# clancylian/retinaface

Hardware: AMD Instinct MI355X
Metric: faces/sec (higher is better)
Workload: dtype f16; 1 GPU; mnet25 fp16 HIP, 448x448, batch 8 per GPU (BASELINE.json configs[1], the metric point); global_batch=8, parallelism=dp1 (image sharding, no data-path collective), tickets_in_flight=96, lanes=3, steps_coalesced_per_launch=32, input=ring of 768 distinct frames per GPU (462 MB, HBM-resident)

## Files before the change

### retinaface_amd/csrc/kernels.hip

```cpp
#include "kernels.h"

#include <atomic>
#include <type_traits>

#include "pack.h"

namespace rf {

typedef float f32x4 __attribute__((ext_vector_type(4)));
typedef _Float16 f16x8 __attribute__((ext_vector_type(8)));

typedef signed char i8x16 __attribute__((ext_vector_type(16)));
typedef int i32x4 __attribute__((ext_vector_type(4)));

template <typename T> struct Vec;
template <> struct Vec<half_t> { static constexpr int N = 8; typedef f16x8 type; };
template <> struct Vec<float> { static constexpr int N = 4; typedef f32x4 type; };
template <> struct Vec<int8_t> { static constexpr int N = 16; typedef i8x16 type; };

template <typename T> __device__ __forceinline__ T to_T(float v);
template <> __device__ __forceinline__ half_t to_T<half_t>(float v) { return (half_t)v; }
template <> __device__ __forceinline__ float to_T<float>(float v) { return v; }
template <> __device__ __forceinline__ int8_t to_T<int8_t>(float v) { return (int8_t)(int)fminf(fmaxf(rintf(v), -127.f), 127.f); }

// ... 2497 lines not shown
    const int lh = L.h, lw = L.w_, hh = lh >> 1, wh = lw >> 1;
    const int n_my = first < ntiles ? (ntiles - 1 - first) / G + 1 : 0;
    const TileStep step(G, L.tiles_x, L.tiles_y);
    auto halo_of = [&](int b) -> T * { return (T *)(smem + (size_t)b * W::BUF_BYTES); };
    auto aux_of = [&](int b) -> T * { return (T *)(smem + (size_t)b * W::BUF_BYTES + W::L_BYTES); };

    int kl[LPW], kc[CPW];
    const int in_ld = L.in_ld;
#pragma unroll
    for (int j = 0; j < LPW; j++) {
        const int s = (wave + 4 * j) * 64 + lane;
        const int row = s / W::CPR, rem = s % W::CPR;
        const int px = rem / W::CPP, ch = rem % W::CPP;
        const bool real = row < HR && px < HC && ch < DPP;
        kl[j] = real ? ((((row * lw + px) * in_ld + ch * VEC) * (int)sizeof(T)) | (px << 26)) : (int)(63u << 26);
    }
#pragma unroll
    for (int j = 0; j < CPW; j++) {
        const int s = (wave + 4 * j) * 64 + lane;
        const int cpix = s / DPP, ch = s % DPP;
        const int cy = cpix / CW, cx = cpix % CW;
        kc[j] = (((cy * wh + cx) * CIN + ch * VEC) * (int)sizeof(T)) | (cx << 26);
    }
    const unsigned lat_bytes = (unsigned)(lh * lw * in_ld - L.in_off) * (unsigned)sizeof(T);
    const unsigned up_bytes = (unsigned)(hh * wh * CIN) * (unsigned)sizeof(T);
    const T *in = L.in + L.in_off;
    auto dma = [&](int tx, int ty, int img, int b) {
        const auto rs = image_rsrc(in + (size_t)img * lh * lw * in_ld, lat_bytes);
        const auto ru = image_rsrc(L.up + (size_t)img * hh * wh * CIN, up_bytes);
        const int iy0 = ty * TH - 1, ix0 = tx * TW - 1;
        const int sbase = (iy0 * lw + ix0) * in_ld * (int)sizeof(T);
        unsigned char *hd = (unsigned char *)halo_of(b), *cd = (unsigned char *)aux_of(b);
#pragma unroll
        for (int j = 0; j < LPW; j++) {
            const int piece = wave + 4 * j;
            const int dx = (int)((unsigned)kl[j] >> 26);
            const unsigned off = (dx != 63 && (unsigned)(ix0 + dx) < (unsigned)lw) ? (unsigned)((kl[j] & 0x03ffffff) + sbase) : kOobOffset;
            if (piece < W::PIECES && piece * 64 + lane < W::SLOTS) lds_dma16(rs, hd + piece * 1024, off);
        }
        const int cy0 = ty * (TH / 2) - 2, cx0 = tx * (TW / 2) - 2;
        const int cbase = (cy0 * wh + cx0) * CIN * (int)sizeof(T);
#pragma unroll
        for (int j = 0; j < CPW; j++) {
            const int piece = wave + 4 * j;
            const int cx = (int)((unsigned)kc[j] >> 26);
            const unsigned off = (unsigned)(cx0 + cx) < (unsigned)wh ? (unsigned)((kc[j] & 0x03ffffff) + cbase) : kOobOffset;
            if (piece < W::CPIECES) lds_dma16(ru, cd + piece * 1024, off);
        }
    };
    T *out0 = L.out0;
    const int ld0 = L.ld0, off0 = L.off0;
    auto store_tile = [&](int b, int img, int oy0, int ox0) {
        constexpr int OPV = 64 / VEC;
        const T *s_res = aux_of(b);
        const auto r0 = image_rsrc(out0 + (size_t)img * lh * lw * ld0 + off0, (unsigned)(lh * lw * ld0 - off0) * (unsigned)sizeof(T));
        const int pbase = oy0 * lw + ox0;
        V v[SPW];
#pragma unroll
        for (int m = 0; m < SPW; m++) { const int i = tid + m * kThreads; v[m] = *(const V *)(s_res + (i / OPV) * LDO + (i % OPV) * VEC); }
#pragma unroll
        for (int m = 0; m < SPW; m++) {
            const int i = tid + m * kThreads;
            const int p = i / OPV, c = (i % OPV) * VEC;
            const int py = p / TW, px = p % TW;
            buf_store16(r0, ox0 + px < lw ? (unsigned)(((pbase + py * lw + px) * ld0 + c) * (int)sizeof(T)) : kOobOffset, v[m]);
        }
    };

    const int wn = wave;
    Frag wst[1][KCH];
    {
        const Frag *wsrc = (const Frag *)L.w + (size_t)wn * KCH * 64 + lane;
#pragma unroll
        for (int kc2 = 0; kc2 < KCH; kc2++) wst[0][kc2] = wsrc[kc2 * 64];
    }
    const f32x4 bias = *(const f32x4 *)(L.b + acc_cout(wn, lane, 0));
    const f32x4 mult = load_mult(L.m, acc_cout(wn, lane, 0));
    const float a_lat = L.a_lat, a_up = L.a_up;
    const bool int_blend = L.int_blend != 0;
    int pbase[NJ];
#pragma unroll
    for (int j = 0; j < NJ; j++) {
        const int p = acc_pixel(j, lane);
        pbase[j] = (p / TW) * ROWP + (p % TW) * LDI;
    }
    int b_lat[W::NBL], b_c0[W::NBL], b_step[W::NBL], b_yx[W::NBL];
#pragma unroll
    for (int m = 0; m < W::NBL; m++) {
        int i = tid + m * 256;
        const bool real = i < HR * HC * DPP;
        i = real ? i : 0;
        const int pix = i / DPP, cv = i % DPP;
        const int dy = pix / HC, dx = pix % HC;
        const int ly = 2 + ((dy - 1) >> 1), lx = 2 + ((dx - 1) >> 1);
        const int sy = ((dy - 1) & 1) ? 1 : -1, sx = ((dx - 1) & 1) ? 1 : -1;
        b_lat[m] = dy * ROWP + dx * LDI + cv * VEC;
        b_c0[m] = (ly * CW + lx) * CIN + cv * VEC;
        b_step[m] = (sy * CW * CIN) * 65536 + (sx * CIN + 32768);
        b_yx[m] = real ? (dy << 8 | dx) : -1;
    }
    __builtin_amdgcn_s_waitcnt(0x0F70);

    TileCoord cur(first, L.tiles_x, L.tiles_y), pf = cur;
#pragma unroll
    for (int d = 0; d < DIST; d++)
        if (d < n_my) { dma(pf.tx, pf.ty, pf.img, d); step.advance(pf); }
    wait_vmcnt<0>();
    lds_barrier();
    int p_img = 0, p_oy0 = 0, p_ox0 = 0;
    for (int k = 0; k < n_my; k++) {
        const int b = k % NBUF;
        const bool st = k > 0, ld = k + DIST < n_my;
        T *s_in_b = halo_of(b);
        T *s_x = aux_of(b);
        const int iy0 = cur.ty * TH - 1, ix0 = cur.tx * TW - 1;
        if (st) store_tile((k - 1) % NBUF, p_img, p_oy0, p_ox0);
        p_img = cur.img; p_oy0 = cur.ty * TH; p_ox0 = cur.tx * TW;
        step.advance(cur);
#pragma unroll
        for (int m = 0; m < W::NBL; m++) {
            if (b_yx[m] < 0) continue;
            const int rs_ = b_step[m] >> 16, cs_ = (b_step[m] & 0xffff) - 32768;
            const V lat = *(const V *)(s_in_b + b_lat[m]);
            const V u0 = *(const V *)(s_x + b_c0[m]), u1 = *(const V *)(s_x + b_c0[m] + cs_);
            const V u2 = *(const V *)(s_x + b_c0[m] + rs_), u3 = *(const V *)(s_x + b_c0[m] + rs_ + cs_);
            const bool ok = (unsigned)(iy0 + (b_yx[m] >> 8)) < (unsigned)lh && (unsigned)(ix0 + (b_yx[m] & 0xff)) < (unsigned)lw;
            *(V *)(s_in_b + b_lat[m]) = upadd_blend<T>(lat, u0, u1, u2, u3, ok, int_blend, a_lat, a_up);
        }
        lds_barrier();
        if (ld) { dma(pf.tx, pf.ty, pf.img, (k + DIST) % NBUF); step.advance(pf); }
        typename M::Acc acc[1][NJ];
#pragma unroll
        for (int j = 0; j < NJ; j++) acc[0][j] = acc_init<T>(bias);
        gemm_stationary<T, 1, NJ, KCH, DEPTH, true>(acc, wst, [&](int j, int kc2) -> Frag {
            const int kb = kc2 * M::K + (lane >> 4) * M::KPL;
            const int tap = kb / CIN, c = kb % CIN;
            const int koff = (tap / 3) * ROWP + (tap % 3) * LDI + c;
            return kb < KTOT ? *(const Frag *)(s_in_b + pbase[j] + koff) : M::zero();
        });
#pragma unroll
        for (int j = 0; j < NJ; j++) store_acc<T, LDO>(s_x, mult, bias, acc[0][j], wn, j, lane, true);
        wait_vmcnt<0>();
        lds_barrier();
    }
    if (n_my > 0) store_tile((n_my - 1) % NBUF, p_img, p_oy0, p_ox0);
}


template <typename T>
static void conv3_ws_launch(hipStream_t s, Conv3Args<T> &a, int nlv, int total_tiles) {
    typedef Conv3WsCfg<T> W;
    auto kern = conv3x3_ws_kernel<T>;
    static std::atomic<int> resident_cache[kMaxDevices] = {};
    const int resident = kernel_residency(resident_cache, kern, W::LDS_BYTES);
    const int want = persistent_grid(total_tiles, resident);
    int grid = 0;
    for (int l = 0; l < 3; l++) {
        Conv3Level<T> &L = a.lv[l];
        if (l >= nlv) { L.gb_begin = 0x7fffffff; L.gsz = 1; L.ntiles = 0; continue; }
        long g = want == total_tiles ? L.ntiles : ((long)L.ntiles * want + total_tiles - 1) / total_tiles;
        if (g < 1) g = 1;
        if (g > L.ntiles) g = L.ntiles;
        L.gb_begin = grid;
        L.gsz = (int)g;
        grid += (int)g;
    }
    hipLaunchKernelGGL(kern, dim3(grid), dim3(kThreads), W::LDS_BYTES, s, a);
}

template <typename T, int CIN, int COUT, int TH, int TW, bool UPADD, bool PADROW>
static void conv3_launch(hipStream_t s, Conv3Args<T> &a, int nlv, int total_tiles) {
    typedef Conv3Cfg<T, CIN, COUT, TH, TW, PADROW> C;
    if constexpr (sizeof(T) <= 2 && CIN == 64 && COUT == 48 && TH == 8 && TW == 8 && !UPADD && PADROW) {
        bool split32 = true;
        for (int l = 0; l < nlv; l++) split32 = split32 && a.lv[l].n0 == 32 && a.lv[l].out1 != nullptr;
        if constexpr (sizeof(T) == 2) {
            if (split32) { conv3_ws_launch<T>(s, a, nlv, total_tiles); return; }
        }
    }
    auto kern = conv3x3_kernel<T, CIN, COUT, TH, TW, UPADD, PADROW>;
    static std::atomic<int> resident_cache[kMaxDevices] = {};
    const int resident = kernel_residency(resident_cache, kern, C::LDS_BYTES);
    const int want = sizeof(T) <= 2 ? persistent_grid(total_tiles, resident) : total_tiles;
    int grid = 0;
    for (int l = 0; l < 3; l++) {
        Conv3Level<T> &L = a.lv[l];
        if (l >= nlv) { L.gb_begin = 0x7fffffff; L.gsz = 1; L.ntiles = 0; continue; }
        long g = want == total_tiles ? L.ntiles : ((long)L.ntiles * want + total_tiles - 1) / total_tiles;
        if (g < 1) g = 1;
        if (g > L.ntiles) g = L.ntiles;
        L.gb_begin = grid;
        L.gsz = (int)g;
        grid += (int)g;
    }
    hipLaunchKernelGGL(kern, dim3(grid), dim3(kThreads), C::LDS_BYTES, s, a);
}

template <typename T, int CIN, int COUT, int TH, int TW, bool PADROW = false>
static TileInfo conv3_dispatch(hipStream_t s, const Conv3Params<T> *p, int nlv, int h, int w) {
    typedef Conv3Cfg<T, CIN, COUT, TH, TW, PADROW> C;
    TileInfo ti{TH, TW, C::LDS_BYTES, ((w + TW - 1) / TW) * ((h + TH - 1) / TH)};
    if (!p) return ti;
    Conv3Args<T> a;
    int total = 0;
    for (int l = 0; l < 3; l++) {
        const Conv3Params<T> &q = p[l < nlv ? l : nlv - 1];
        int tiles_x = (q.w_ + TW - 1) / TW, tiles_y = (q.h + TH - 1) / TH;
        a.lv[l] = Conv3Level<T>{q.in, q.up, q.w, q.b, q.m, q.out0, q.out1, q.in_ld, q.in_off, q.ld0, q.off0, q.n0, q.ld1, q.off1,
                                q.h, q.w_, tiles_x, tiles_y, q.n * tiles_x * tiles_y, 0, 1, q.a_lat, q.a_up,
                                (sizeof(T) == 1 && q.a_lat == 1.f && q.a_up == 1.f && !q.blend_fp32) ? 1 : 0};
        if (l < nlv) total += q.n * tiles_x * tiles_y;
    }
    if (p[0].up) {
        if constexpr (CIN == 64 && COUT == 64) conv3_launch<T, CIN, COUT, TH, TW, true, PADROW>(s, a, nlv, total);
        else throw LaunchUnsupported("fused upsample + add: only the 64 -> 64 aggregation conv has a kernel instance");
    } else {
        conv3_launch<T, CIN, COUT, TH, TW, false, PADROW>(s, a, nlv, total);
    }
    return ti;
}

template <typename T>
static void conv3_up_ws_launch(hipStream_t s, const Conv3Params<T> &q) {
    typedef Conv3UpWsCfg<T> W;
    auto kern = conv3x3_up_dma_kernel<T>;
    static std::atomic<int> resident_cache[kMaxDevices] = {};
    const int dev = launch_device();
    int resident = resident_cache[dev].load(std::memory_order_acquire);
    if (!resident) {
        set_max_lds(kern, W::LDS_BYTES);
        int nb = 0;
        if (hipOccupancyMaxActiveBlocksPerMultiprocessor(&nb, (const void *)kern, kThreads, W::LDS_BYTES) != hipSuccess || nb < 1) nb = 1;
        resident = nb;
        resident_cache[dev].store(resident, std::memory_order_release);
    }
    const int tiles_x = (q.w_ + 7) / 8, tiles_y = (q.h + 7) / 8;
    Conv3Args<T> a;
    for (int l = 0; l < 3; l++)
        a.lv[l] = Conv3Level<T>{q.in, q.up, q.w, q.b, q.m, q.out0, q.out1, q.in_ld, q.in_off, q.ld0, q.off0, q.n0, q.ld1, q.off1,
                                q.h, q.w_, tiles_x, tiles_y, q.n * tiles_x * tiles_y, 0, 1, q.a_lat, q.a_up,
                                (sizeof(T) == 1 && q.a_lat == 1.f && q.a_up == 1.f && !q.blend_fp32) ? 1 : 0};
    const int total = q.n * tiles_x * tiles_y;
    if (total == 0) return;
    a.lv[0].gsz = persistent_grid(total, resident);
    hipLaunchKernelGGL(kern, dim3(a.lv[0].gsz), dim3(kThreads), W::LDS_BYTES, s, a);
}

template <typename T>
static TileInfo conv3_select(hipStream_t s, const Conv3Params<T> *p, int nlv, int cin, int cout, int h, int w) {
    if constexpr (sizeof(T) <= 2) {
        const bool up_ws = sizeof(T) == 2 && p && (long)p[0].h * p[0].w_ >= 48 * 48;
        if (p && nlv == 1 && p[0].up && cin == 64 && cout == 64 && up_ws && p[0].h % 2 == 0 && p[0].w_ % 2 == 0 &&
            p[0].n0 == 64 && p[0].in_ld == 64) {
            conv3_up_ws_launch<T>(s, p[0]);
            return TileInfo{8, 8, Conv3UpWsCfg<T>::LDS_BYTES, ((w + 7) / 8) * ((h + 7) / 8)};
        }
        if (cin == 64 && cout == 64) return conv3_dispatch<T, 64, 64, 4, 8, true>(s, p, nlv, h, w);
        if (cin == 64 && cout == 48) return conv3_dispatch<T, 64, 48, 8, 8, true>(s, p, nlv, h, w);
        return TileInfo{0, 0, 0, 0};
    }
    else {
        const bool small = nlv == 1 && (size_t)h * w <= 32 * 32;
        if (cin == 64 && cout == 64)
            return conv3_dispatch<T, 64, 64, 4, 8>(s, p, nlv, h, w);
        if (cin == 16 && cout == 32)
            return small ? conv3_dispatch<T, 16, 32, 4, 8>(s, p, nlv, h, w) : conv3_dispatch<T, 16, 32, 8, 8>(s, p, nlv, h, w);
        if (cin == 64 && cout == 48) return conv3_dispatch<T, 64, 48, 8, 8>(s, p, nlv, h, w);
        if (cin == 16 && cout == 16) return conv3_dispatch<T, 16, 16, 8, 8>(s, p, nlv, h, w);
    }
    return TileInfo{0, 0, 0, 0};
}

template <typename T> void launch_conv3x3(hipStream_t s, const Conv3Params<T> *levels, int nlevels) {
    if (nlevels < 1 || nlevels > 3) throw LaunchUnsupported("conv3x3: 1..3 levels per launch");
    for (int l = 1; l < nlevels; l++)
        if (levels[l].cin != levels[0].cin || levels[l].cout != levels[0].cout || levels[l].up)
            throw LaunchUnsupported("conv3x3: the levels of one launch must share (cin, cout) and have no fused upsample");
    TileInfo ti = conv3_select<T>(s, levels, nlevels, levels[0].cin, levels[0].cout, levels[0].h, levels[0].w_);
    if (ti.th == 0) throw LaunchUnsupported("no 3x3 kernel instance for this (cin, cout)");
}
template <typename T> TileInfo conv3x3_tile_info(int cin, int cout, int h, int w) {
    return conv3_select<T>(nullptr, nullptr, 1, cin, cout, h, w);
}
template void launch_conv3x3<half_t>(hipStream_t, const Conv3Params<half_t> *, int);
template void launch_conv3x3<float>(hipStream_t, const Conv3Params<float> *, int);
template void launch_conv3x3<int8_t>(hipStream_t, const Conv3Params<int8_t> *, int);
template TileInfo conv3x3_tile_info<half_t>(int, int, int, int);
template TileInfo conv3x3_tile_info<float>(int, int, int, int);
template TileInfo conv3x3_tile_info<int8_t>(int, int, int, int);

template <typename T> struct SshTailCfg {
    typedef Mma<T> M;
    static constexpr int VEC = Vec<T>::N;
    static constexpr int TH = 8, TW = 8, P = TH * TW;
    static constexpr int R1 = TW + 2, N1 = (TH + 2) * R1, PT1 = (N1 + 15) / 16;
    static constexpr int HC = TW + 4, NH = (TH + 4) * HC;
    static constexpr int LDI = lds_row<T>(16);
    static constexpr int LDO = lds_row<T>(32);
    static constexpr int KTOT = 9 * 16, KCH = (KTOT + M::K - 1) / M::K;
    static constexpr int CPV = 16 / VEC;
    static constexpr int STAGE_ITEMS = NH * CPV, NPF = (STAGE_ITEMS + kThreads - 1) / kThreads;
    static constexpr size_t IN_BYTES = sizeof(T) * (size_t)(NH * LDI), MID_BYTES = sizeof(T) * (size_t)(PT1 * 16 * LDI),
                            OUT_BYTES = sizeof(T) * (size_t)(P * LDO);
    static constexpr size_t LDS_BYTES = IN_BYTES + MID_BYTES + 2 * OUT_BYTES;
    static_assert(IN_BYTES % 16 == 0 && MID_BYTES % 16 == 0, "LDS carve must stay 16-byte aligned");
    static constexpr int OCC = 4;
};

template <typename T>
struct SshTailLevel {
    const T *in; const T *wb; const float *bb; const float *mb; const T *wc; const float *bc; const float *mc; T *cat;
    int h, w_, tiles_x, tiles_y, ntiles, gb_begin, gsz;
};
template <typename T> struct SshTailArgs { SshTailLevel<T> lv[3]; };

template <typename T, typename ACC>
__device__ __forceinline__ uint2 pack_acc(f32x4 mult, f32x4 bv, ACC acc) {
    uint2 h = {0u, 0u};
    if constexpr (sizeof(T) == 2) {
        h.x = pack_f16((float)acc[0], (float)acc[1], true);
        h.y = pack_f16((float)acc[2], (float)acc[3], true);
    } else {
        static_assert(sizeof(T) == 1, "fp16 / int8 engines only");
#pragma unroll
        for (int r = 0; r < 4; r++)
            h.x = __builtin_amdgcn_cvt_pk_u8_f32(RF_RNDNE(__builtin_amdgcn_fmed3f(fmaf((float)acc[r], mult[r], bv[r]), 0.f, 127.f)), r, h.x);
    }
    return h;
}
template <typename T> __device__ __forceinline__ void store_packed4(T *dst, uint2 h) {
    if constexpr (sizeof(T) == 2) *(uint2 *)dst = h;
    else *(uint32_t *)dst = h.x;
}

template <typename T>
__global__ __launch_bounds__(kThreads, SshTailCfg<T>::OCC) void ssh_tail_kernel(SshTailArgs<T> a) {
    typedef SshTailCfg<T> C;
    typedef typename Vec<T>::type V;
    typedef Mma<T> M;
    typedef typename M::Frag Frag;
    constexpr int VEC = C::VEC, TH = C::TH, TW = C::TW, P = C::P, R1 = C::R1, N1 = C::N1, PT1 = C::PT1, HC = C::HC;
    constexpr int LDI = C::LDI, LDO = C::LDO, KTOT = C::KTOT, KCH = C::KCH, CPV = C::CPV, NPF = C::NPF;
    extern __shared__ __attribute__((aligned(16))) unsigned char smem[];
    T *s_in = (T *)smem;
    T *s_mid = (T *)(smem + C::IN_BYTES);
    T *s_out = (T *)(smem + C::IN_BYTES + C::MID_BYTES);

    const int tid = threadIdx.x, lane = tid & 63, wave = tid >> 6;
    const int gbid = xcd_remap(blockIdx.x, gridDim.x);
    const int lvl = (gbid >= a.lv[1].gb_begin ? 1 : 0) + (gbid >= a.lv[2].gb_begin ? 1 : 0);
    const SshTailLevel<T> &L = a.lv[lvl];
    const int first = gbid - L.gb_begin, G = L.gsz, ntiles = L.ntiles;
    const int lh = L.h, lw = L.w_;
    const int kg = lane >> 4;

    const int ctb = wave & 1, ptb0 = wave >> 1;
    Frag wb[1][KCH], wc[1][KCH];
    {
        const Frag *sb = (const Frag *)L.wb + (size_t)ctb * KCH * 64 + lane, *sc = (const Frag *)L.wc + lane;
#pragma unroll
        for (int kc = 0; kc < KCH; kc++) { wb[0][kc] = sb[kc * 64]; wc[0][kc] = sc[kc * 64]; }
    }
    const f32x4 bias_b = *(const f32x4 *)(L.bb + acc_cout(ctb, lane, 0)), mult_b = load_mult(L.mb, acc_cout(ctb, lane, 0));
    const f32x4 bias_c = *(const f32x4 *)(L.bc + acc_cout(0, lane, 0)), mult_c = load_mult(L.mc, acc_cout(0, lane, 0));

    int pb1[4], ryx1[4];
#pragma unroll
    for (int i = 0; i < 4; i++) {
        const int pt = ptb0 + 2 * i;
        int p = pt * 16 + (lane & 15);
        const bool real = pt < PT1 && p < N1;
        p = real ? p : N1 - 1;
        const int ry = p / R1, rx = p % R1;
        pb1[i] = (ry * HC + rx) * LDI;
        ryx1[i] = real ? (ry << 8 | rx) : -1;
    }
    const int p2 = wave * 16 + (lane & 15);
    const int pb2 = ((p2 / TW) * R1 + p2 % TW) * LDI;

    V pre[NPF];
    int koff[NPF], kdx[NPF];
#pragma unroll
    for (int k = 0; k < NPF; k++) {
        int i = tid + k * kThreads;
        i = i < C::STAGE_ITEMS ? i : C::STAGE_ITEMS - 1;
        const int pix = i / CPV, cv = i % CPV;
        koff[k] = (((pix / HC) * lw + pix % HC) * 16 + cv * VEC) * (int)sizeof(T);
        kdx[k] = pix % HC;
    }
    const unsigned in_img_bytes = (unsigned)(lh * lw * 16) * (unsigned)sizeof(T);
    auto fetch = [&](int tx, int ty, int img) {
        const auto rs = image_rsrc(L.in + (size_t)img * lh * lw * 16, in_img_bytes);
        const int iy0 = ty * TH - 2, ix0 = tx * TW - 2;
        const int sbase = (iy0 * lw + ix0) * 16 * (int)sizeof(T);
#pragma unroll
        for (int k = 0; k < NPF; k++) {
            const unsigned off = (unsigned)(ix0 + kdx[k]) < (unsigned)lw ? (unsigned)(koff[k] + sbase) : kOobOffset;
            pre[k] = buf_load16<V>(rs, off);
        }
    };
    auto store_tile = [&](const T *s_res, int img, int oy0, int ox0) {
        constexpr int OPV = 32 / VEC;
        const auto ro = image_rsrc(L.cat + (size_t)img * lh * lw * 64 + 32, (unsigned)(lh * lw * 64 - 32) * (unsigned)sizeof(T));
        const int pbase = oy0 * lw + ox0;
        for (int i = tid; i < P * OPV; i += kThreads) {
            const int p = i / OPV, cv = i % OPV;
            const int py = p / TW, px = p % TW;
            const unsigned off = ox0 + px < lw ? (unsigned)(((pbase + py * lw + px) * 64 + cv * VEC) * (int)sizeof(T)) : kOobOffset;
            buf_store16(ro, off, *(const V *)(s_res + p * LDO + cv * VEC));
        }
    };
    const TileStep step(G, L.tiles_x, L.tiles_y);
    TileCoord cur(first, L.tiles_x, L.tiles_y), nxt = cur;
    step.advance(nxt);
    if (first < ntiles) fetch(cur.tx, cur.ty, cur.img);
    __builtin_amdgcn_s_waitcnt(0x0F70);

    auto xf_tap = [&](int kc, int rowp) -> int {
        const int kb = kc * M::K + kg * M::KPL;
        const int tap = kb / 16, c = kb % 16;
        return kb < KTOT ? (tap / 3) * rowp + (tap % 3) * LDI + c : -1;
    };

    int p_img = -1, p_oy0 = 0, p_ox0 = 0;
    int buf = 0;
    constexpr int O_ELEMS = (int)(C::OUT_BYTES / sizeof(T));
    for (int t = first; t < ntiles; t += G) {
        const int oy0 = cur.ty * TH, ox0 = cur.tx * TW, img = cur.img;
        T *const s_out_b = s_out + buf * O_ELEMS;
#pragma unroll
        for (int k = 0; k < NPF; k++) {
            const int i = tid + k * kThreads;
            if (i < C::STAGE_ITEMS) *(V *)(s_in + (i / CPV) * LDI + (i % CPV) * VEC) = pre[k];
        }
        if (t + G < ntiles) fetch(nxt.tx, nxt.ty, nxt.img);
        cur = nxt;
        step.advance(nxt);
        __syncthreads();
        if (p_img >= 0) store_tile(s_out + (buf ^ 1) * O_ELEMS, p_img, p_oy0, p_ox0);
        p_img = img; p_oy0 = oy0; p_ox0 = ox0;

#pragma unroll
        for (int half = 0; half < 2; half++) {
            typename M::Acc acc[1][2];
#pragma unroll
            for (int j = 0; j < 2; j++) acc[0][j] = acc_init<T>(bias_b);
            gemm_stationary<T, 1, 2, KCH, 2>(acc, wb, [&](int j, int kc) -> Frag {
                const int o = xf_tap(kc, HC * LDI);
                return o >= 0 ? *(const Frag *)(s_in + pb1[2 * half + j] + o) : M::zero();
            });
#pragma unroll
            for (int jj = 0; jj < 2; jj++) {
                const int j = 2 * half + jj;
                if (ryx1[j] < 0) continue;
                const int ry = ryx1[j] >> 8, rx = ryx1[j] & 0xff;
                const uint2 h = pack_acc<T>(mult_b, bias_b, acc[0][jj]);
                if (ctb == 0) {
                    if ((unsigned)(ry - 1) < (unsigned)TH && (unsigned)(rx - 1) < (unsigned)TW)
                        store_packed4<T>(s_out_b + ((ry - 1) * TW + rx - 1) * LDO + kg * 4, h);
                } else {
                    const int y = oy0 - 1 + ry, x = ox0 - 1 + rx;
                    const bool inside = (unsigned)y < (unsigned)lh && (unsigned)x < (unsigned)lw;
                    const uint2 z = {0u, 0u};
                    store_packed4<T>(s_mid + (ry * R1 + rx) * LDI + kg * 4, inside ? h : z);
                }
            }
        }
        __syncthreads();

        {
            typename M::Acc acc[1][1];
            acc[0][0] = acc_init<T>(bias_c);
            gemm_stationary<T, 1, 1, KCH, 2>(acc, wc, [&](int, int kc) -> Frag {
                const int o = xf_tap(kc, R1 * LDI);
                return o >= 0 ? *(const Frag *)(s_mid + pb2 + o) : M::zero();
            });
            store_packed4<T>(s_out_b + p2 * LDO + 16 + kg * 4, pack_acc<T>(mult_c, bias_c, acc[0][0]));
        }
        buf ^= 1;
    }
    __syncthreads();
    if (p_img >= 0) store_tile(s_out + (buf ^ 1) * O_ELEMS, p_img, p_oy0, p_ox0);
}

template <typename T> void launch_ssh_tail(hipStream_t s, const SshTailParams<T> *levels, int nlevels) {
    typedef SshTailCfg<T> C;
    if (nlevels < 1 || nlevels > 3) throw LaunchUnsupported("ssh tail: 1..3 levels per launch");
    auto kern = ssh_tail_kernel<T>;
    static std::atomic<int> resident_cache[kMaxDevices] = {};
    const int resident = kernel_residency(resident_cache, kern, C::LDS_BYTES);
    SshTailArgs<T> a;
    int total = 0;
    for (int l = 0; l < 3; l++) {
        const SshTailParams<T> &q = levels[l < nlevels ? l : nlevels - 1];
        const int tiles_x = (q.w_ + C::TW - 1) / C::TW, tiles_y = (q.h + C::TH - 1) / C::TH;
        a.lv[l] = SshTailLevel<T>{q.in, q.wb, q.bb, q.mb, q.wc, q.bc, q.mc, q.cat, q.h, q.w_, tiles_x, tiles_y, q.n * tiles_x * tiles_y, 0, 1};
        if (l < nlevels) total += q.n * tiles_x * tiles_y;
    }
    if (total == 0) return;
    const int want = persistent_grid(total, resident);
    int grid = 0;
    for (int l = 0; l < 3; l++) {
        SshTailLevel<T> &L = a.lv[l];
        if (l >= nlevels) { L.gb_begin = 0x7fffffff; L.gsz = 1; L.ntiles = 0; continue; }
        long g = want == total ? L.ntiles : ((long)L.ntiles * want + total - 1) / total;
        if (g < 1) g = 1;
        if (g > L.ntiles) g = L.ntiles;
        L.gb_begin = grid; L.gsz = (int)g; grid += (int)g;
    }
    hipLaunchKernelGGL(kern, dim3(grid), dim3(kThreads), C::LDS_BYTES, s, a);
}
template void launch_ssh_tail<half_t>(hipStream_t, const SshTailParams<half_t> *, int);
template void launch_ssh_tail<int8_t>(hipStream_t, const SshTailParams<int8_t> *, int);

constexpr int HEAD_P = 64;

__device__ __forceinline__ void decode_anchor(const float *__restrict__ o , int a, int na,
                                              float ax1, float ay1, float ax2, float ay2, int net_w, int net_h,
                                              float conf, int anchor_index, Candidate *dst) {
#pragma clang fp contract(off)
    const float width = ax2 - ax1 + 1.f;
    const float height = ay2 - ay1 + 1.f;
    const float ctr_x = (float)((double)ax1 + 0.5 * ((double)width - 1.0));
    const float ctr_y = (float)((double)ay1 + 0.5 * ((double)height - 1.0));
    const float *d = o + 2 * na + a * 4;
    const float pred_ctr_x = d[0] * width + ctr_x;
    const float pred_ctr_y = d[1] * height + ctr_y;
    const float pred_w = expf(d[2]) * width;
    const float pred_h = expf(d[3]) * height;
    float x1 = (float)((double)pred_ctr_x - 0.5 * ((double)pred_w - 1.0));
    float y1 = (float)((double)pred_ctr_y - 0.5 * ((double)pred_h - 1.0));
    float x2 = (float)((double)pred_ctr_x + 0.5 * ((double)pred_w - 1.0));
    float y2 = (float)((double)pred_ctr_y + 0.5 * ((double)pred_h - 1.0));
    if (x1 < 0) x1 = 0;
    if (y1 < 0) y1 = 0;
    if (x2 > (float)(net_w - 1)) x2 = (float)(net_w - 1);
    if (y2 > (float)(net_h - 1)) y2 = (float)(net_h - 1);
    dst->score = conf;
    dst->x1 = x1; dst->y1 = y1; dst->x2 = x2; dst->y2 = y2;
    const float *l = o + 6 * na + a * 10;
#pragma unroll
    for (int k = 0; k < 5; k++) {
        dst->px[k] = l[2 * k] * width + ctr_x;
        dst->py[k] = l[2 * k + 1] * height + ctr_y;
    }
    dst->anchor = anchor_index;
}

template <typename T>
struct HeadLevel {
    const T *in; const T *w; const float *b; const float *m;
    float *dump_prob, *dump_bbox, *dump_lmk;
    float base[4][4];
    int hw, w_, stride, anchor_offset, blocks_per_image, blk_begin;
};
template <typename T>
struct HeadArgs {
    HeadLevel<T> lv[3];
    int net_h, net_w;
    const RunParams *params;
    Candidate *cand; int *cand_count; int cap;
    int nblk;
};

template <typename T, int NA>
__global__ __launch_bounds__(kThreads) void head_kernel(HeadArgs<T> a) {
    typedef typename Vec<T>::type V;
    typedef Mma<T> M;
    constexpr int VEC = Vec<T>::N, CIN = 64, COUT = 16 * NA, P = HEAD_P, LDA = lds_row<T>(CIN), LDOH = COUT + 1;
    constexpr int CPV = CIN / VEC;
    __shared__ __attribute__((aligned(16))) T s_a[P * LDA];
    __shared__ float s_o[P * LDOH];

    const int tid = threadIdx.x;
    const int lane = tid & 63, wave = tid >> 6;
    const int gbid = xcd_remap(blockIdx.x, a.nblk);
    const int lvl = (gbid >= a.lv[1].blk_begin ? 1 : 0) + (gbid >= a.lv[2].blk_begin ? 1 : 0);
    const HeadLevel<T> &L = a.lv[lvl];
    const int bid = gbid - L.blk_begin;
    const int img = bid / L.blocks_per_image;
    const int p0 = (bid % L.blocks_per_image) * P;
    const int hw = L.hw;

    constexpr int NT = COUT / 16, PT = P / 16;
    typedef WaveSplit<NT, PT> WS;
    constexpr int KCH1 = CIN / M::K, KCH = sizeof(T) == 2 ? 2 * KCH1 : KCH1;
    const int wn = wave % WS::WN, wp = wave / WS::WN;
    GemmPipe<T, 1, WS::NJ, KCH, WS::WN> pipe;
    pipe.init(L.w, wn, lane);
    const float threshold = a.params->threshold;
    const f32x4 bias = *(const f32x4 *)(L.b + acc_cout(wn, lane, 0));
    const f32x4 mult = load_mult(L.m, acc_cout(wn, lane, 0));

    const T *inb = L.in + (size_t)img * hw * CIN;
    for (int i = tid; i < P * CPV; i += kThreads) {
        int p = i / CPV, cv = i % CPV;
        V v = vzero<V, VEC>();
        if (p0 + p < hw) v = *(const V *)(inb + (size_t)(p0 + p) * CIN + cv * VEC);
        *(V *)(s_a + p * LDA + cv * VEC) = v;
    }
    __syncthreads();

    typename M::Acc acc[1][WS::NJ];
#pragma unroll
    for (int j = 0; j < WS::NJ; j++) acc[0][j] = vzero<typename M::Acc, 4>();
    pipe.run(acc, [&](int j, int kc) -> typename M::Frag {
        const int kb = (kc % KCH1) * M::K + (lane >> 4) * M::KPL;
        return *(const typename M::Frag *)(s_a + acc_pixel(wp + j * WS::WP, lane) * LDA + kb);
    });
#pragma unroll
    for (int j = 0; j < WS::NJ; j++) {
        const int p = acc_pixel(wp + j * WS::WP, lane);
        const int c0 = acc_cout(wn, lane, 0);
#pragma unroll
        for (int r = 0; r < 4; r++) s_o[p * LDOH + c0 + r] = fmaf((float)acc[0][j][r], mult[r], bias[r]);
    }
    __syncthreads();

    if (tid < NA * P) {
        const int p = tid % P, an = tid / P;
        const int gp = p0 + p;
        if (gp < hw) {
            const float *o = s_o + p * LDOH;
            const float s0 = o[an], s1 = o[NA + an];
            const float m = fmaxf(s0, s1);
            const float e0 = expf(s0 - m), e1 = expf(s1 - m);
            const float sum = e0 + e1;
            const float conf = e1 / sum;
            if (L.dump_prob) {
                const size_t shw = (size_t)hw;
                L.dump_prob[((size_t)img * 2 * NA + an) * shw + gp] = e0 / sum;
                L.dump_prob[((size_t)img * 2 * NA + NA + an) * shw + gp] = conf;
#pragma unroll
                for (int c = 0; c < 4; c++) L.dump_bbox[((size_t)img * 4 * NA + an * 4 + c) * shw + gp] = o[2 * NA + an * 4 + c];
#pragma unroll
                for (int c = 0; c < 10; c++) L.dump_lmk[((size_t)img * 10 * NA + an * 10 + c) * shw + gp] = o[6 * NA + an * 10 + c];
            }
            if (conf > threshold) {
                const int iy = gp / L.w_, ix = gp % L.w_;
                const float sx = (float)(ix * L.stride), sy = (float)(iy * L.stride);
                const int slot = atomicAdd(&a.cand_count[img], 1);
                if (slot < a.cap)
                    decode_anchor(o, an, NA, L.base[an][0] + sx, L.base[an][1] + sy, L.base[an][2] + sx, L.base[an][3] + sy,
                                  a.net_w, a.net_h, conf, L.anchor_offset + an * hw + gp,
                                  a.cand + (size_t)img * a.cap + slot);
            }
        }
    }
}

template <typename T> void launch_head(hipStream_t s, const HeadParams<T> *levels, int nlevels) {
    if (nlevels < 1 || nlevels > 3) throw LaunchUnsupported("heads: 1..3 strides per launch");
    HeadArgs<T> a;
    int blk = 0;
    for (int l = 0; l < 3; l++) {
        const HeadParams<T> &p = levels[l < nlevels ? l : nlevels - 1];
        HeadLevel<T> &L = a.lv[l];
        L.in = p.in; L.w = p.w; L.b = p.b; L.m = p.m;
        L.dump_prob = p.dump_prob; L.dump_bbox = p.dump_bbox; L.dump_lmk = p.dump_lmk;
        for (int i = 0; i < 4; i++) for (int j = 0; j < 4; j++) L.base[i][j] = p.base[i][j];
        L.hw = p.h * p.w_; L.w_ = p.w_; L.stride = p.stride; L.anchor_offset = p.anchor_offset;
        L.blocks_per_image = (L.hw + HEAD_P - 1) / HEAD_P;
        L.blk_begin = l < nlevels ? blk : 0x7fffffff;
        if (l < nlevels) blk += p.n * L.blocks_per_image;
    }
    const HeadParams<T> &p0 = levels[0];
    a.net_h = p0.net_h; a.net_w = p0.net_w; a.params = p0.params;
    a.cand = p0.cand; a.cand_count = p0.cand_count; a.cap = p0.cap;
    a.nblk = blk;
    if (p0.num_anchors == 0 || a.nblk == 0) return;
    if (p0.num_anchors == 4) hipLaunchKernelGGL((head_kernel<T, 4>), dim3(a.nblk), dim3(kThreads), 0, s, a);
    else if (p0.num_anchors == 2) hipLaunchKernelGGL((head_kernel<T, 2>), dim3(a.nblk), dim3(kThreads), 0, s, a);
    else throw LaunchUnsupported("heads: 2 or 4 anchors per cell");
}
template void launch_head<half_t>(hipStream_t, const HeadParams<half_t> *, int);
template void launch_head<float>(hipStream_t, const HeadParams<float> *, int);
template void launch_head<int8_t>(hipStream_t, const HeadParams<int8_t> *, int);

constexpr int NMS_THREADS = 256;

__global__ __launch_bounds__(NMS_THREADS) void nms_kernel(NmsParams a) {
#pragma clang fp contract(off)
    extern __shared__ __attribute__((aligned(16))) unsigned char smem[];
    const int cap = a.cap;
    unsigned long long *s_key = (unsigned long long *)smem;
    float4 *s_box = (float4 *)(s_key + cap);
    int *s_slot = (int *)(s_box + cap);
    int *s_kept = s_slot + cap;
    unsigned char *s_alive = (unsigned char *)(s_kept + a.max_det);

    const int tid = threadIdx.x;
    const int img = blockIdx.x;
    const Candidate *cand = a.cand + (size_t)img * cap;
    const float thr = a.params->nms_threshold;
    const int n_found = a.cand_count[img];
    int n = n_found;
    if (n > cap) n = cap;
    const bool small = n <= 64;
    if (small && tid >= 64) return;
    const int nthr = small ? 64 : NMS_THREADS;
    if (n <= 256) {
        for (int i = tid; i < n; i += nthr) {
            const unsigned int sbits = __float_as_uint(cand[i].score);
            s_key[i] = ((unsigned long long)(~sbits) << 32) | (unsigned int)cand[i].anchor;
        }
        __syncthreads();
        for (int i = tid; i < n; i += nthr) {
            const unsigned long long ki = s_key[i];
            int rank = 0;
            for (int j = 0; j < n; j++) { const unsigned long long kj = s_key[j]; rank += (kj < ki || (kj == ki && j < i)) ? 1 : 0; }
            s_slot[rank] = i;
        }
        __syncthreads();
    } else {
        int npow = 512;
        while (npow < n) npow <<= 1;
        for (int i = tid; i < npow; i += nthr) {
            unsigned long long key = ~0ull;
            if (i < n) {
                const unsigned int sbits = __float_as_uint(cand[i].score);
                key = ((unsigned long long)(~sbits) << 32) | (unsigned int)cand[i].anchor;
            }
            s_key[i] = key;
            s_slot[i] = i;
        }
        __syncthreads();
        for (int k = 2; k <= npow; k <<= 1) {
            for (int j = k >> 1; j > 0; j >>= 1) {
                for (int i = tid; i < npow; i += nthr) {
                    const int l = i ^ j;
                    if (l > i) {
                        const unsigned long long ki = s_key[i], kl = s_key[l];
                        const bool up = (i & k) == 0;
                        if ((ki > kl) == up) {
                            s_key[i] = kl; s_key[l] = ki;
                            const int t = s_slot[i]; s_slot[i] = s_slot[l]; s_slot[l] = t;
                        }
                    }
                }
                __syncthreads();
            }
        }
    }
    for (int i = tid; i < n; i += nthr) {
        const Candidate *c = cand + s_slot[i];
        s_box[i] = make_float4(c->x1, c->y1, c->x2, c->y2);
        s_alive[i] = 1;
    }
    __syncthreads();

    const int lane = tid & 63;
    int kept = 0;
    for (int base = 0; base < n; base += 64) {
        const int idx = base + lane;
        unsigned long long mask = __ballot(idx < n && s_alive[idx]);
        while (mask) {
            const int sel = base + __ffsll((long long)mask) - 1;
            if (tid == 0 && kept < a.max_det) s_kept[kept] = sel;
            kept++;
            const float4 sb = s_box[sel];
            const float area1 = (sb.z - sb.x + 1) * (sb.w - sb.y + 1);
            for (int i = sel + 1 + tid; i < n; i += nthr) {
                if (!s_alive[i]) continue;
                const float4 bi = s_box[i];
                const float x = fmaxf(sb.x, bi.x);
                const float y = fmaxf(sb.y, bi.y);
                const float w = fminf(sb.z, bi.z) - x + 1;
                const float h = fminf(sb.w, bi.w) - y + 1;
                if (w <= 0 || h <= 0) continue;
                const float area2 = (bi.z - bi.x + 1) * (bi.w - bi.y + 1);
                const float inter = w * h;
                if (inter / (area1 + area2 - inter) > thr) s_alive[i] = 0;
            }
            __syncthreads();
            const unsigned long long later = (sel - base) >= 63 ? 0ull : (~0ull << (sel - base + 1));
            mask = __ballot(idx < n && s_alive[idx]) & later;
        }
    }
    __syncthreads();
    const int nout = kept < a.max_det ? kept : a.max_det;
// ... 2648 lines not shown
```

Before: 421,800 faces/s.

## Rebalance SSH tail work: only compute conv-b halo, move inner ctb0 tile after sync

The fused SSH tail kernel now runs the first-stage conv over the full halo region only for the output-channel half that feeds the second conv. The other half is computed only on the 8x8 interior, after the barrier, by waves 2-3 while waves 0-1 run the second conv. The staged input is double-buffered in LDS so the next tile's prefetch store does not overwrite input still being read in the second phase. The wave index is made uniform via readfirstlane. Together these drop the redundant halo MMAs and balance work across waves, at the cost of more LDS per block, which may reduce occupancy.

```diff
diff --git a/retinaface_amd/csrc/kernels.hip b/retinaface_amd/csrc/kernels.hip
--- a/retinaface_amd/csrc/kernels.hip
+++ b/retinaface_amd/csrc/kernels.hip
@@ -2823,7 +2823,7 @@
     static constexpr int STAGE_ITEMS = NH * CPV, NPF = (STAGE_ITEMS + kThreads - 1) / kThreads;
     static constexpr size_t IN_BYTES = sizeof(T) * (size_t)(NH * LDI), MID_BYTES = sizeof(T) * (size_t)(PT1 * 16 * LDI),
                             OUT_BYTES = sizeof(T) * (size_t)(P * LDO);
-    static constexpr size_t LDS_BYTES = IN_BYTES + MID_BYTES + 2 * OUT_BYTES;
+    static constexpr size_t LDS_BYTES = 2 * IN_BYTES + MID_BYTES + 2 * OUT_BYTES;
     static_assert(IN_BYTES % 16 == 0 && MID_BYTES % 16 == 0, "LDS carve must stay 16-byte aligned");
     static constexpr int OCC = 4;
 };
@@ -2864,10 +2864,11 @@
     constexpr int LDI = C::LDI, LDO = C::LDO, KTOT = C::KTOT, KCH = C::KCH, CPV = C::CPV, NPF = C::NPF;
     extern __shared__ __attribute__((aligned(16))) unsigned char smem[];
     T *s_in = (T *)smem;
-    T *s_mid = (T *)(smem + C::IN_BYTES);
-    T *s_out = (T *)(smem + C::IN_BYTES + C::MID_BYTES);
-
-    const int tid = threadIdx.x, lane = tid & 63, wave = tid >> 6;
+    T *s_mid = (T *)(smem + 2 * C::IN_BYTES);
+    T *s_out = (T *)(smem + 2 * C::IN_BYTES + C::MID_BYTES);
+
+    const int tid = threadIdx.x, lane = tid & 63;
+    const int wave = __builtin_amdgcn_readfirstlane(tid >> 6);
     const int gbid = xcd_remap(blockIdx.x, gridDim.x);
     const int lvl = (gbid >= a.lv[1].gb_begin ? 1 : 0) + (gbid >= a.lv[2].gb_begin ? 1 : 0);
     const SshTailLevel<T> &L = a.lv[lvl];
@@ -2875,20 +2876,23 @@
     const int lh = L.h, lw = L.w_;
     const int kg = lane >> 4;
 
-    const int ctb = wave & 1, ptb0 = wave >> 1;
-    Frag wb[1][KCH], wc[1][KCH];
+    const bool side_c = wave < 2;
+    Frag wb[1][KCH], w2[1][KCH];
     {
-        const Frag *sb = (const Frag *)L.wb + (size_t)ctb * KCH * 64 + lane, *sc = (const Frag *)L.wc + lane;
-#pragma unroll
-        for (int kc = 0; kc < KCH; kc++) { wb[0][kc] = sb[kc * 64]; wc[0][kc] = sc[kc * 64]; }
-    }
-    const f32x4 bias_b = *(const f32x4 *)(L.bb + acc_cout(ctb, lane, 0)), mult_b = load_mult(L.mb, acc_cout(ctb, lane, 0));
-    const f32x4 bias_c = *(const f32x4 *)(L.bc + acc_cout(0, lane, 0)), mult_c = load_mult(L.mc, acc_cout(0, lane, 0));
-
-    int pb1[4], ryx1[4];
-#pragma unroll
-    for (int i = 0; i < 4; i++) {
-        const int pt = ptb0 + 2 * i;
+        const Frag *sb = (const Frag *)L.wb + (size_t)KCH * 64 + lane, *s2 = (const Frag *)(side_c ? L.wc : L.wb) + lane;
+#pragma unroll
+        for (int kc = 0; kc < KCH; kc++) { wb[0][kc] = sb[kc * 64]; w2[0][kc] = s2[kc * 64]; }
+    }
+    const f32x4 bias_b = *(const f32x4 *)(L.bb + acc_cout(1, lane, 0)), mult_b = load_mult(L.mb, acc_cout(1, lane, 0));
+    const f32x4 bias_2 = *(const f32x4 *)((side_c ? L.bc : L.bb) + acc_cout(0, lane, 0));
+    const f32x4 mult_2 = load_mult(side_c ? L.mc : L.mb, acc_cout(0, lane, 0));
+
+    static_assert(PT1 > 4 && PT1 <= 8 && P == 64, "unit map: one or two region pixel tiles and two tile pixel tiles per wave");
+    const bool pair1 = wave + 4 < PT1;
+    int pb1[2], ryx1[2];
+#pragma unroll
+    for (int i = 0; i < 2; i++) {
+        const int pt = wave + 4 * i;
         int p = pt * 16 + (lane & 15);
         const bool real = pt < PT1 && p < N1;
         p = real ? p : N1 - 1;
@@ -2896,8 +2900,13 @@
         pb1[i] = (ry * HC + rx) * LDI;
         ryx1[i] = real ? (ry << 8 | rx) : -1;
     }
-    const int p2 = wave * 16 + (lane & 15);
-    const int pb2 = ((p2 / TW) * R1 + p2 % TW) * LDI;
+    int po2[2], pb2[2];
+#pragma unroll
+    for (int j = 0; j < 2; j++) {
+        const int p = ((wave & 1) * 2 + j) * 16 + (lane & 15), py = p / TW, px = p % TW;
+        po2[j] = p * LDO + (side_c ? 16 : 0) + kg * 4;
+        pb2[j] = side_c ? (py * R1 + px) * LDI : ((py + 1) * HC + px + 1) * LDI;
+    }
 
     V pre[NPF];
     int koff[NPF], kdx[NPF];
@@ -2945,14 +2954,15 @@
 
     int p_img = -1, p_oy0 = 0, p_ox0 = 0;
     int buf = 0;
-    constexpr int O_ELEMS = (int)(C::OUT_BYTES / sizeof(T));
+    constexpr int I_ELEMS = (int)(C::IN_BYTES / sizeof(T)), O_ELEMS = (int)(C::OUT_BYTES / sizeof(T));
     for (int t = first; t < ntiles; t += G) {
         const int oy0 = cur.ty * TH, ox0 = cur.tx * TW, img = cur.img;
+        T *const s_in_b = s_in + buf * I_ELEMS;
         T *const s_out_b = s_out + buf * O_ELEMS;
 #pragma unroll
         for (int k = 0; k < NPF; k++) {
             const int i = tid + k * kThreads;
-            if (i < C::STAGE_ITEMS) *(V *)(s_in + (i / CPV) * LDI + (i % CPV) * VEC) = pre[k];
+            if (i < C::STAGE_ITEMS) *(V *)(s_in_b + (i / CPV) * LDI + (i % CPV) * VEC) = pre[k];
         }
         if (t + G < ntiles) fetch(nxt.tx, nxt.ty, nxt.img);
         cur = nxt;
@@ -2961,42 +2971,46 @@
         if (p_img >= 0) store_tile(s_out + (buf ^ 1) * O_ELEMS, p_img, p_oy0, p_ox0);
         p_img = img; p_oy0 = oy0; p_ox0 = ox0;
 
-#pragma unroll
-        for (int half = 0; half < 2; half++) {
-            typename M::Acc acc[1][2];
-#pragma unroll
-            for (int j = 0; j < 2; j++) acc[0][j] = acc_init<T>(bias_b);
-            gemm_stationary<T, 1, 2, KCH, 2>(acc, wb, [&](int j, int kc) -> Frag {
+        auto conv3_1 = [&](auto nj) {
+            constexpr int NJ = decltype(nj)::value;
+            typename M::Acc acc[1][NJ];
+#pragma unroll
+            for (int j = 0; j < NJ; j++) acc[0][j] = acc_init<T>(bias_b);
+            gemm_stationary<T, 1, NJ, KCH, 2>(acc, wb, [&](int j, int kc) -> Frag {
                 const int o = xf_tap(kc, HC * LDI);
-                return o >= 0 ? *(const Frag *)(s_in + pb1[2 * half + j] + o) : M::zero();
+                return o >= 0 ? *(const Frag *)(s_in_b + pb1[j] + o) : M::zero();
             });
 #pragma unroll
-            for (int jj = 0; jj < 2; jj++) {
-                const int j = 2 * half + jj;
+            for (int j = 0; j < NJ; j++) {
                 if (ryx1[j] < 0) continue;
                 const int ry = ryx1[j] >> 8, rx = ryx1[j] & 0xff;
-                const uint2 h = pack_acc<T>(mult_b, bias_b, acc[0][jj]);
-                if (ctb == 0) {
-                    if ((unsigned)(ry - 1) < (unsigned)TH && (unsigned)(rx - 1) < (unsigned)TW)
-                        store_packed4<T>(s_out_b + ((ry - 1) * TW + rx - 1) * LDO + kg * 4, h);
-                } else {
-                    const int y = oy0 - 1 + ry, x = ox0 - 1 + rx;
-                    const bool inside = (unsigned)y < (unsigned)lh && (unsigned)x < (unsigned)lw;
-                    const uint2 z = {0u, 0u};
-                    store_packed4<T>(s_mid + (ry * R1 + rx) * LDI + kg * 4, inside ? h : z);
-                }
-            }
-        }
+                const uint2 h = pack_acc<T>(mult_b, bias_b, acc[0][j]);
+                const int y = oy0 - 1 + ry, x = ox0 - 1 + rx;
+                const bool inside = (unsigned)y < (unsigned)lh && (unsigned)x < (unsigned)lw;
+                const uint2 z = {0u, 0u};
+                store_packed4<T>(s_mid + (ry * R1 + rx) * LDI + kg * 4, inside ? h : z);
+            }
+        };
+        if (pair1) conv3_1(std::integral_constant<int, 2>());
+        else conv3_1(std::integral_constant<int, 1>());
         __syncthreads();
 
         {
-            typename M::Acc acc[1][1];
-            acc[0][0] = acc_init<T>(bias_c);
-            gemm_stationary<T, 1, 1, KCH, 2>(acc, wc, [&](int, int kc) -> Frag {
-                const int o = xf_tap(kc, R1 * LDI);
-                return o >= 0 ? *(const Frag *)(s_mid + pb2 + o) : M::zero();
-            });
-            store_packed4<T>(s_out_b + p2 * LDO + 16 + kg * 4, pack_acc<T>(mult_c, bias_c, acc[0][0]));
+            typename M::Acc acc[1][2];
+#pragma unroll
+            for (int j = 0; j < 2; j++) acc[0][j] = acc_init<T>(bias_2);
+            if (side_c)
+                gemm_stationary<T, 1, 2, KCH, 2>(acc, w2, [&](int j, int kc) -> Frag {
+                    const int o = xf_tap(kc, R1 * LDI);
+                    return o >= 0 ? *(const Frag *)(s_mid + pb2[j] + o) : M::zero();
+                });
+            else
+                gemm_stationary<T, 1, 2, KCH, 2>(acc, w2, [&](int j, int kc) -> Frag {
+                    const int o = xf_tap(kc, HC * LDI);
+                    return o >= 0 ? *(const Frag *)(s_in_b + pb2[j] + o) : M::zero();
+                });
+#pragma unroll
+            for (int j = 0; j < 2; j++) store_packed4<T>(s_out_b + po2[j], pack_acc<T>(mult_2, bias_2, acc[0][j]));
         }
         buf ^= 1;
     }
```

After: 418,300 faces/s. Within noise of the previous version (-0.8%).
